# adajel/knp-emi-fenics-x

Hardware: AMD Instinct MI355X
Metric: assembled dofs/s (volume + membrane-facet assembly + membrane ODE sweep) per timestep; 3D idealized mesh, fp64 (higher is better)
Workload: dtype f64

## Files before the change

knp-emi-fenics-x_amd/csrc/kernels_assemble.hip:

```cpp
#include "knpemi_internal.h"

#define KN_ROW_STORE(v, p) __builtin_nontemporal_store((v), (p))

namespace {

__device__ __forceinline__ int logical_block(int bid, int nb) {
  const int q = nb >> 3, r = nb & 7, xcd = bid & 7, idx = bid >> 3;
  return xcd * q + (xcd < r ? xcd : r) + idx;
}

struct Rec {
  double x, y, z, c[KN_MAXK], phi;
};

__device__ __forceinline__ Rec load_rec(const double* __restrict__ VR, int v) {
  const double4* p = reinterpret_cast<const double4*>(VR) + 2 * (size_t)v;
  const double4 a = p[0], b = p[1];
  Rec r;
  r.x = a.x; r.y = a.y; r.z = a.z; r.c[0] = b.x; r.c[1] = b.y; r.c[2] = b.z; r.c[3] = a.w; r.phi = b.w;
  return r;
}

template <int NF>
__device__ __forceinline__ double facet_measure(const Rec (&p)[NF]) {
// ... 1361 lines not shown
    }
  }
#pragma unroll
  for (int m = 1; m < KN_MEM_LQ; m <<= 1)
#pragma unroll
    for (int a = 0; a < NF; ++a)
#pragma unroll
      for (int k = 0; k < KN_MAXK - 1; ++k) acc[a][k] += __shfl_xor(acc[a][k], m);
  if (live && lq == 0) {
#pragma unroll
    for (int a = 0; a < NF; ++a)
#pragma unroll
      for (int k = 0; k < KN_MAXK - 1; ++k)
        if (k < KS) D.gam_e[(size_t)KS * pos[a] + k] = acc[a][k];
  }
}

template <int NF>
__global__ __launch_bounds__(256) void knp_membrane_kernel(KnDev D, const KnConsts* __restrict__ Cp, int splitting) {
  extern __shared__ double qt[];
  knp_membrane_block<NF>(D, *Cp, splitting, logical_block(blockIdx.x, gridDim.x), nullptr, qt);
}

template <int NF>
__global__ __launch_bounds__(256) void emi_writeback_membrane_kernel(KnDev D, const KnConsts* __restrict__ Cp, int splitting,
                                                                     int nbm, const double* __restrict__ x, int n,
                                                                     const double* __restrict__ part, int np, double inv_n,
                                                                     double* __restrict__ mean_out) {
  extern __shared__ double qt[];
  if ((int)blockIdx.x < nbm) {
    knp_membrane_block<NF>(D, *Cp, splitting, logical_block(blockIdx.x, nbm), x, qt);
    return;
  }
  const int vb = blockIdx.x - nbm, nvb = gridDim.x - nbm;
  int i = vb * 256 + threadIdx.x;
  double xi = i < n ? x[i] : 0.0;
  double mean = 0.0;
  if (np > 0) {
    double v0 = 0.0, v1 = 0.0, v2 = 0.0, v3 = 0.0;
    const int t = threadIdx.x;
    if (t < np) v0 = part[t];
    if (t + 256 < np) v1 = part[t + 256];
    if (t + 512 < np) v2 = part[t + 512];
    if (t + 768 < np) v3 = part[t + 768];
    double sum = ((v0 + v1) + v2) + v3;
#pragma unroll
    for (int m = 32; m >= 1; m >>= 1) sum += __shfl_xor(sum, m);
    __shared__ double sh[4];
    if ((t & 63) == 0) sh[t >> 6] = sum;
    __syncthreads();
    mean = ((sh[0] + sh[1]) + (sh[2] + sh[3])) * inv_n;
    if (vb == 0 && t == 0 && mean_out) *mean_out = mean;
  }
  while (i < n) {
    D.VR[(size_t)i * KN_REC + 7] = xi - mean;
    i += nvb * 256;
    if (i < n) xi = x[i];
// ... 166 lines not shown
                            double* __restrict__ buf) {
  const int i = blockIdx.x * blockDim.x + threadIdx.x;
  if (i >= n) return;
  const int g = idx[i];
  if (kind == 0) {
    double* rec = D.VR + (size_t)g * KN_REC + 3;
    double* b = buf + (size_t)i * 5;
#pragma unroll
    for (int c = 0; c < 5; ++c) {
      if (pack) b[c] = rec[c];
      else rec[c] = b[c];
    }
  } else {
    const int w = 1 + KN_MAXK * n_slots;
    double* b = buf + (size_t)i * w;
    if (pack) b[0] = D.phiM[g];
    else D.phiM[g] = b[0];
    for (int c = 0; c < KN_MAXK * n_slots; ++c) {
      double* f = D.Ich + (size_t)c * D.NQtot + g;
      if (pack) b[1 + c] = *f;
      else *f = b[1 + c];
    }
  }
}

template <int NF, int LPR>
__global__ __launch_bounds__(256) void emi_membrane_rhs_kernel(KnDev D, const KnConsts* __restrict__ Cp, int splitting) {
  const KnConsts& C = *Cp;
  const int t = blockIdx.x * blockDim.x + threadIdx.x;
  const int mm = t / LPR, sub = t % LPR;
  const bool live = mm < D.M;
  const int m = live ? mm : D.M - 1;
  const int g = D.mrow[m];
  const bool cell_side = g >= C.voff[1];
  double gam = 0.0;
  for (int e = D.mptr[m] + sub; e < D.mptr[m + 1]; e += LPR) {
    const int ms = D.me_model[e];
    if (ms < 0) continue;
    gam += (cell_side ? 1.0 : -1.0) * C.C_phi * emi_membrane_entry_rhs<NF>(D, C, e, ms, splitting);
  }
#pragma unroll
  for (int k = 1; k < LPR; k <<= 1) gam += __shfl_xor(gam, k);
  if (live && sub == 0) D.b_emi[g] = D.b_emi[g] + gam;
}

int check_launch(const char* what) {
  hipError_t e = hipGetLastError();
  if (e != hipSuccess) {
    kn_set_error(std::string(what) + ": " + hipGetErrorString(e));
    return KNPEMI_EHIP;
  }
  return KNPEMI_OK;
}

template <class K>
int set_lds_limit(K kernel, size_t bytes) {
  if (bytes > 64 * 1024) {
    hipError_t e = hipFuncSetAttribute(reinterpret_cast<const void*>(kernel),
                                       hipFuncAttributeMaxDynamicSharedMemorySize, (int)bytes);
    if (e != hipSuccess) {
      kn_set_error(std::string("hipFuncSetAttribute(max dynamic LDS): ") + hipGetErrorString(e));
      return KNPEMI_EHIP;
    }
  }
  return KNPEMI_OK;
}
// ... 152 lines not shown
  const KnDev& D = h->dev;
  dim3 grid((n_entries + 255) / 256), block(256);
  const int v_cells = h->voff[1];
  if (h->NF == 2) hipLaunchKernelGGL(membrane_mass_kernel<2>, grid, block, 0, h->stream, D, n_entries, v_cells, d_entry_row, d_out);
  else if (h->NF == 3) hipLaunchKernelGGL(membrane_mass_kernel<3>, grid, block, 0, h->stream, D, n_entries, v_cells, d_entry_row, d_out);
  else hipLaunchKernelGGL(membrane_mass_kernel<4>, grid, block, 0, h->stream, D, n_entries, v_cells, d_entry_row, d_out);
  return check_launch("membrane_mass_kernel");
}

int kn_launch_knp_membrane(knpemi_handle* h, int flags) {
  const KnDev& D = h->dev;
  if (D.nftot == 0) return KNPEMI_OK;
  const int split = (flags & KNPEMI_NO_SPLITTING) ? 0 : 1;
  const int NF = h->NF;
  const size_t lds = (size_t)D.nq_gamma * (1 + NF + (NF == 4 ? 2 * NF : 0)) * sizeof(double);
  dim3 grid((2 * (size_t)D.nftot * KN_MEM_LQ + 255) / 256), block(256);
  KnProfScope prof(h, KNPEMI_K_KNP_MEMBRANE);
  if (NF == 2) hipLaunchKernelGGL((knp_membrane_kernel<2>), grid, block, lds, h->cur, D, h->d_consts, split);
  else if (NF == 3) hipLaunchKernelGGL((knp_membrane_kernel<3>), grid, block, lds, h->cur, D, h->d_consts, split);
  else hipLaunchKernelGGL((knp_membrane_kernel<4>), grid, block, lds, h->cur, D, h->d_consts, split);
  return check_launch("knp_membrane_kernel");
}

int kn_launch_emi_writeback_membrane(knpemi_handle* h, const double* x, const double* part, int np, double inv_n, double* mean_out) {
  const KnDev& D = h->dev;
  const int n = D.Ntot;
  if (n == 0) return KNPEMI_OK;
  const int split = (h->emi_flags & KNPEMI_NO_SPLITTING) ? 0 : 1;
  const int NF = h->NF;
  const size_t lds = (size_t)D.nq_gamma * (1 + NF + (NF == 4 ? 2 * NF : 0)) * sizeof(double);
  const int nbm = (int)((2 * (size_t)D.nftot * KN_MEM_LQ + 255) / 256);
  const int nbv = std::max(1, std::min(1024, (n + 255) / 256));
  dim3 grid(nbm + nbv), block(256);
  KnProfScope prof(h, KNPEMI_K_KNP_MEMBRANE);
  if (NF == 2) hipLaunchKernelGGL((emi_writeback_membrane_kernel<2>), grid, block, lds, h->cur, D, h->d_consts, split, nbm, x, n, part, np, inv_n, mean_out);
  else if (NF == 3) hipLaunchKernelGGL((emi_writeback_membrane_kernel<3>), grid, block, lds, h->cur, D, h->d_consts, split, nbm, x, n, part, np, inv_n, mean_out);
  else hipLaunchKernelGGL((emi_writeback_membrane_kernel<4>), grid, block, lds, h->cur, D, h->d_consts, split, nbm, x, n, part, np, inv_n, mean_out);
  return check_launch("emi_writeback_membrane_kernel");
}

int kn_launch_knp_membrane_pre(knpemi_handle* h, int flags) {
  const KnDev& D = h->dev;
  if (D.nftot == 0) return KNPEMI_OK;
  const int split = (flags & KNPEMI_NO_SPLITTING) ? 0 : 1;
  const int NF = h->NF;
  const size_t lds = (size_t)D.nq_gamma * (1 + NF + (NF == 4 ? 2 * NF : 0)) * sizeof(double);
  dim3 grid((2 * D.nftot + 255) / 256), block(256);
  KnProfScope prof(h, KNPEMI_K_KNP_MEMBRANE);
  if (NF == 2) hipLaunchKernelGGL((knp_membrane_pre_kernel<2>), grid, block, lds, h->cur, D, h->d_consts, split);
  else if (NF == 3) hipLaunchKernelGGL((knp_membrane_pre_kernel<3>), grid, block, lds, h->cur, D, h->d_consts, split);
  else hipLaunchKernelGGL((knp_membrane_pre_kernel<4>), grid, block, lds, h->cur, D, h->d_consts, split);
  return check_launch("knp_membrane_pre_kernel");
}

int kn_launch_emi_membrane_rhs(knpemi_handle* h, int flags) {
  const KnDev& D = h->dev;
  if (D.M == 0) return KNPEMI_OK;
  const int split = (flags & KNPEMI_NO_SPLITTING) ? 0 : 1;
  const int lpr = h->lpr;
  dim3 grid(((size_t)D.M * lpr + 255) / 256), block(256);
// ... 62 lines not shown
```

knp-emi-fenics-x_amd/csrc/knpemi_api.hip:

```cpp
#include <algorithm>
#include <array>
#include <cstdlib>
#include <cstring>
#include <numeric>

#include "knpemi_internal.h"

static thread_local std::string g_err;
void kn_set_error(const std::string& msg) { g_err = msg; }

extern "C" const char* knpemi_last_error(void) { return g_err.c_str(); }

extern "C" int knpemi_device_count(void) {
  int n = 0;
  if (hipGetDeviceCount(&n) != hipSuccess) return 0;
  return n;
}

namespace {

template <class T>
int dev_upload(knpemi_handle* h, const std::vector<T>& v, const T** out) {
  void* p = nullptr;
  size_t bytes = std::max<size_t>(v.size(), 1) * sizeof(T);
// ... 1072 lines not shown
  const int nq = h->n_q[sub], ne = h->n_vert[0], ni = h->n_vert[sub];
  if (nq == 0) return KNPEMI_OK;
  if ((size_t)ne + ni + 2 * (size_t)nq > h->stage_len) return fail(KNPEMI_EINVAL, "knpemi_trace: staging buffer too small");
  KN_HIP(hipSetDevice(h->device));
  double* de = h->d_stage;
  double* di = de + ne;
  double* qe = di + ni;
  double* qi = qe + nq;
  KN_HIP(hipMemcpyAsync(de, u_e, (size_t)ne * sizeof(double), hipMemcpyHostToDevice, h->stream));
  KN_HIP(hipMemcpyAsync(di, u_i, (size_t)ni * sizeof(double), hipMemcpyHostToDevice, h->stream));
  int rc = kn_launch_trace(h, de, di, sub, qe, qi);
  if (rc) return rc;
  KN_HIP(hipMemcpyAsync(q_e, qe, (size_t)nq * sizeof(double), hipMemcpyDeviceToHost, h->stream));
  KN_HIP(hipMemcpyAsync(q_i, qi, (size_t)nq * sizeof(double), hipMemcpyDeviceToHost, h->stream));
  KN_HIP(hipStreamSynchronize(h->stream));
  return KNPEMI_OK;
}

extern "C" int knpemi_assemble_emi(knpemi_handle* h, int flags) {
  if (!h) return fail(KNPEMI_EINVAL, "null handle");
  if (!h->have_params) return fail(KNPEMI_EINVAL, "knpemi_assemble_emi: knpemi_set_params not called");
  KN_HIP(hipSetDevice(h->device));
  h->emi_flags = flags;
  if (flags & KNPEMI_ON_AUX_STREAM) {
    KN_HIP(hipEventRecord(h->ev_fork, h->stream));
    KN_HIP(hipStreamWaitEvent(h->aux, h->ev_fork, 0));
    h->cur = h->aux;
    int rc = kn_launch_emi_rows(h, flags);
    h->cur = h->stream;
    if (rc) return rc;
    KN_HIP(hipEventRecord(h->ev_join, h->aux));
    return KNPEMI_OK;
  }
  return kn_launch_emi_rows(h, flags);
}

extern "C" int knpemi_join(knpemi_handle* h) {
  if (!h) return fail(KNPEMI_EINVAL, "null handle");
  KN_HIP(hipSetDevice(h->device));
  KN_HIP(hipStreamWaitEvent(h->stream, h->ev_join, 0));
  KN_HIP(hipStreamWaitEvent(h->stream, h->ev_join2, 0));
  return KNPEMI_OK;
}

extern "C" int knpemi_assemble_emi_membrane_rhs(knpemi_handle* h, int flags) {
  if (!h) return fail(KNPEMI_EINVAL, "null handle");
  if (!h->have_params) return fail(KNPEMI_EINVAL, "knpemi_assemble_emi_membrane_rhs: knpemi_set_params not called");
  KN_HIP(hipSetDevice(h->device));
  return kn_launch_emi_membrane_rhs(h, flags);
}

extern "C" int knpemi_assemble_knp_membrane_early(knpemi_handle* h, int flags) {
  if (!h) return fail(KNPEMI_EINVAL, "null handle");
  if (!h->have_params) return fail(KNPEMI_EINVAL, "knpemi_assemble_knp_membrane_early: knpemi_set_params not called");
  KN_HIP(hipSetDevice(h->device));
  int rc;
  if (flags & KNPEMI_ON_AUX_STREAM) {
    KN_HIP(hipEventRecord(h->ev_pre_fork, h->stream));
    KN_HIP(hipStreamWaitEvent(h->aux, h->ev_pre_fork, 0));
    h->cur = h->aux;
    rc = kn_launch_knp_membrane_pre(h, flags);
    h->cur = h->stream;
    if (rc) return rc;
    KN_HIP(hipEventRecord(h->ev_pre, h->aux));
    h->pre_pending = 1;
    return KNPEMI_OK;
  }
  return kn_launch_knp_membrane_pre(h, flags);
}

extern "C" int knpemi_assemble_knp(knpemi_handle* h, int flags) {
  if (!h) return fail(KNPEMI_EINVAL, "null handle");
  if (!h->have_params) return fail(KNPEMI_EINVAL, "knpemi_assemble_knp: knpemi_set_params not called");
  KN_HIP(hipSetDevice(h->device));
  KN_HIP(hipStreamWaitEvent(h->stream, h->ev_join, 0));
  KN_HIP(hipStreamWaitEvent(h->stream, h->ev_join2, 0));
  if (flags & KNPEMI_MEMBRANE_EARLY) {
    if (h->pre_pending) {
      KN_HIP(hipStreamWaitEvent(h->stream, h->ev_pre, 0));
      h->pre_pending = 0;
    }
    return kn_launch_knp_rows(h, flags);
  }
  if (!h->fuse_membrane) {
    const int split = (flags & KNPEMI_NO_SPLITTING) ? 0 : 1;
    if (!kn_gam_current(h, split)) {
      int rc = kn_launch_knp_membrane(h, flags);
      if (rc) return rc;
    }
  }
  return kn_launch_knp_rows(h, flags);
}

extern "C" int knpemi_solve_emi(knpemi_handle* h, double rtol, double atol, int maxit, int* iters, double* relres) {
  if (!h) return fail(KNPEMI_EINVAL, "null handle");
  if (!(rtol >= 0) || !(atol >= 0) || maxit < 0) return fail(KNPEMI_EINVAL, "knpemi_solve_emi: bad tolerances");
  kn_inputs_changed(h);
  KN_HIP(hipSetDevice(h->device));
  KN_HIP(hipStreamWaitEvent(h->stream, h->ev_join, 0));
  KN_HIP(hipStreamWaitEvent(h->stream, h->ev_join2, 0));
  return kn_solve_emi(h, rtol, atol, maxit, iters, relres);
}

extern "C" int knpemi_solve_knp(knpemi_handle* h, double rtol, double atol, int maxit, int* iters, double* relres) {
  if (!h) return fail(KNPEMI_EINVAL, "null handle");
  if (!(rtol >= 0) || !(atol >= 0) || maxit < 0) return fail(KNPEMI_EINVAL, "knpemi_solve_knp: bad tolerances");
  kn_inputs_changed(h);
  KN_HIP(hipSetDevice(h->device));
  KN_HIP(hipStreamWaitEvent(h->stream, h->ev_join, 0));
  KN_HIP(hipStreamWaitEvent(h->stream, h->ev_join2, 0));
  return kn_solve_knp(h, rtol, atol, maxit, iters, relres);
}

extern "C" int knpemi_extrapolate_guess(knpemi_handle* h, int which) {
  if (!h) return fail(KNPEMI_EINVAL, "null handle");
  if (which != KNPEMI_B_EMI && which != KNPEMI_B_KNP) return fail(KNPEMI_EINVAL, "knpemi_extrapolate_guess: unknown system");
  kn_inputs_changed(h);
  KN_HIP(hipSetDevice(h->device));
  return kn_extrapolate_guess(h, which);
}

extern "C" int knpemi_solver_setup(knpemi_handle* h, int which, int precond, double theta) {
  if (!h) return fail(KNPEMI_EINVAL, "null handle");
  if (which != KNPEMI_B_EMI && which != KNPEMI_B_KNP) return fail(KNPEMI_EINVAL, "knpemi_solver_setup: unknown system");
  if (precond != KNPEMI_PC_JACOBI && precond != KNPEMI_PC_AMG)
    return fail(KNPEMI_EINVAL, "knpemi_solver_setup: unknown preconditioner");
  KnAmg& G = which == KNPEMI_B_EMI ? h->amg_emi : h->amg_knp;
  (which == KNPEMI_B_EMI ? h->pc_emi : h->pc_knp) = precond;
  G.cfg.theta = theta > 0 ? theta : 0.08;
  G.built = false;
  return KNPEMI_OK;
}

// ... 59 lines not shown
}

extern "C" int knpemi_get_csr_values(knpemi_handle* h, int which, double* vals) {
  if (!h || !vals) return fail(KNPEMI_EINVAL, "knpemi_get_csr_values: null argument");
  const double* src; size_t n;
  if (which == KNPEMI_A_EMI) { src = h->dev.A_emi; n = h->dev.nnz; }
  else if (which == KNPEMI_P_EMI) { src = h->dev.P_emi; n = h->dev.nnz; }
  else if (which == KNPEMI_A_KNP) { src = h->dev.A_knp; n = (size_t)(h->K - 1) * h->dev.nnzL; }
  else return fail(KNPEMI_EINVAL, "knpemi_get_csr_values: unknown matrix");
  KN_HIP(hipSetDevice(h->device));
  KN_HIP(hipMemcpyAsync(vals, src, n * sizeof(double), hipMemcpyDeviceToHost, h->stream));
  KN_HIP(hipStreamSynchronize(h->stream));
  return KNPEMI_OK;
}

extern "C" int knpemi_set_csr_values(knpemi_handle* h, int which, const double* vals) {
  if (!h || !vals) return fail(KNPEMI_EINVAL, "knpemi_set_csr_values: null argument");
  double* dst; size_t n;
  if (which == KNPEMI_A_EMI) { dst = h->dev.A_emi; n = h->dev.nnz; }
  else if (which == KNPEMI_P_EMI) { dst = h->dev.P_emi; n = h->dev.nnz; }
  else if (which == KNPEMI_A_KNP) { dst = h->dev.A_knp; n = (size_t)(h->K - 1) * h->dev.nnzL; }
  else return fail(KNPEMI_EINVAL, "knpemi_set_csr_values: unknown matrix");
  KN_HIP(hipSetDevice(h->device));
  KN_HIP(hipStreamWaitEvent(h->stream, h->ev_join, 0));
  KN_HIP(hipMemcpyAsync(dst, vals, n * sizeof(double), hipMemcpyHostToDevice, h->stream));
  KN_HIP(hipStreamSynchronize(h->stream));
  return KNPEMI_OK;
}

extern "C" int knpemi_set_rhs(knpemi_handle* h, int which, const double* b) {
  if (!h || !b) return fail(KNPEMI_EINVAL, "knpemi_set_rhs: null argument");
  double* dst; size_t n;
  if (which == KNPEMI_B_EMI) { dst = h->dev.b_emi; n = h->dev.Ntot; }
  else if (which == KNPEMI_B_KNP) { dst = h->dev.b_knp; n = (size_t)(h->K - 1) * h->dev.Ntot; }
  else return fail(KNPEMI_EINVAL, "knpemi_set_rhs: unknown vector");
  KN_HIP(hipSetDevice(h->device));
  KN_HIP(hipStreamWaitEvent(h->stream, h->ev_join, 0));
  KN_HIP(hipMemcpyAsync(dst, b, n * sizeof(double), hipMemcpyHostToDevice, h->stream));
  KN_HIP(hipStreamSynchronize(h->stream));
  return KNPEMI_OK;
}

extern "C" int knpemi_device_rhs(knpemi_handle* h, int which, const double** b) {
  if (!h || !b) return fail(KNPEMI_EINVAL, "null argument");
  if (which == KNPEMI_B_EMI) *b = h->dev.b_emi;
  else if (which == KNPEMI_B_KNP) *b = h->dev.b_knp;
  else return fail(KNPEMI_EINVAL, "knpemi_device_rhs: unknown vector");
  return KNPEMI_OK;
}

extern "C" int knpemi_get_rhs(knpemi_handle* h, int which, double* b) {
  if (!h || !b) return fail(KNPEMI_EINVAL, "knpemi_get_rhs: null argument");
  const double* src; size_t n;
  if (which == KNPEMI_B_EMI) { src = h->dev.b_emi; n = h->dev.Ntot; }
  else if (which == KNPEMI_B_KNP) { src = h->dev.b_knp; n = (size_t)(h->K - 1) * h->dev.Ntot; }
  else return fail(KNPEMI_EINVAL, "knpemi_get_rhs: unknown vector");
  KN_HIP(hipSetDevice(h->device));
  KN_HIP(hipMemcpyAsync(b, src, n * sizeof(double), hipMemcpyDeviceToHost, h->stream));
  KN_HIP(hipStreamSynchronize(h->stream));
  return KNPEMI_OK;
}

extern "C" int knpemi_set_solution(knpemi_handle* h, int which, const double* x, int on_device) {
  if (!h || !x) return fail(KNPEMI_EINVAL, "knpemi_set_solution: null argument");
  kn_inputs_changed(h);
  KN_HIP(hipSetDevice(h->device));
  const hipMemcpyKind kind = on_device ? hipMemcpyDeviceToDevice : hipMemcpyHostToDevice;
  KnDev& D = h->dev;
  if (which == KNPEMI_B_EMI) {
    const double* src = x;
    if (!on_device) {
      KN_HIP(hipMemcpyAsync(h->d_stage, x, (size_t)D.Ntot * sizeof(double), kind, h->stream));
      src = h->d_stage;
    }
    if (on_device && h->fold_membrane && h->have_params && !h->fuse_membrane && !h->dist.on) {
      KN_HIP(hipStreamWaitEvent(h->stream, h->ev_join, 0));
      KN_HIP(hipStreamWaitEvent(h->stream, h->ev_join2, 0));
      if (int rc = kn_launch_emi_writeback_membrane(h, src, nullptr, 0, 0.0, nullptr)) return rc;
      kn_gam_formed(h, (h->emi_flags & KNPEMI_NO_SPLITTING) ? 0 : 1);
    } else if (int rc = kn_launch_field_scatter(h, src, D.VR + 7, D.Ntot, KN_REC)) return rc;
  } else if (which == KNPEMI_B_KNP) {
    const int KS = h->K - 1;
    if (on_device) {
      if (!h->have_params) return fail(KNPEMI_EINVAL, "knpemi_set_solution: knpemi_set_params not called");
      int rc = h->fuse_update ? kn_launch_knp_writeback_update(h, x) : kn_launch_knp_order(h, const_cast<double*>(x), 0);
      if (rc) return rc;
    } else
    for (int s = 0; s < h->n_sub; ++s)
      for (int k = 0; k < KS; ++k) {
        const size_t nv = h->n_vert[s];
        if (!nv) continue;
        KN_HIP(hipMemcpyAsync(D.csol + (size_t)k * D.Ntot + h->voff[s],
                              x + (size_t)KS * h->voff[s] + (size_t)k * nv, nv * sizeof(double), kind, h->stream));
      }
  } else return fail(KNPEMI_EINVAL, "knpemi_set_solution: unknown system");
  if (!on_device && which == KNPEMI_B_KNP && h->fuse_update) {
    if (!h->have_params) return fail(KNPEMI_EINVAL, "knpemi_set_solution: knpemi_set_params not called");
    int rc = kn_launch_update_pde(h);
    if (rc) return rc;
  }
  if (!on_device) KN_HIP(hipStreamSynchronize(h->stream));
  return KNPEMI_OK;
}

extern "C" int knpemi_get_solution(knpemi_handle* h, int which, double* x) {
// ... 160 lines not shown
  KnOdeModel& m = h->ode[slot];
  for (int i = 0; i < 3 * h->K; ++i)
    if (ion_param[i] < 0 || ion_param[i] >= m.n_params)
      return fail(KNPEMI_EINVAL, "knpemi_ode_step: parameter index out of range");
  if (v_index < 0 || v_index >= m.n_states) return fail(KNPEMI_EINVAL, "knpemi_ode_step: bad V index");
  const bool fixed = m.method != KNPEMI_ODE_LSODA;
  if (!(dt > 0) || (!fixed && (!(rtol >= 0) || !(atol >= 0) || (rtol == 0 && atol == 0))))
    return fail(KNPEMI_EINVAL, "knpemi_ode_step: bad dt / tolerances");
  if (h->ode_only && (flags & (KNPEMI_ODE_SET_TRACES | KNPEMI_ODE_SET_V)))
    return fail(KNPEMI_EINVAL, "knpemi_ode_step: a handle of knpemi_ode_create has no PDE fields to read");
  kn_inputs_changed(h);
  KN_HIP(hipSetDevice(h->device));
  if (flags & (KNPEMI_ODE_ON_AUX_STREAM | KNPEMI_ODE_ON_AUX2_STREAM)) {
    const bool second = (flags & KNPEMI_ODE_ON_AUX2_STREAM) != 0;
    hipStream_t side = second ? h->aux2 : h->aux;
    KN_HIP(hipEventRecord(h->ev_fork, h->stream));
    KN_HIP(hipStreamWaitEvent(side, h->ev_fork, 0));
    h->cur = side;
    int rc = fixed ? kn_launch_ode_fixed_step(h, slot, t0, dt, flags, ion_param, v_index)
                   : kn_launch_ode_step(h, slot, t0, dt, rtol, atol, flags, ion_param, v_index);
    h->cur = h->stream;
    if (rc) return rc;
    KN_HIP(hipEventRecord(second ? h->ev_join2 : h->ev_join, side));
    return KNPEMI_OK;
  }
  if (fixed) return kn_launch_ode_fixed_step(h, slot, t0, dt, flags, ion_param, v_index);
  return kn_launch_ode_step(h, slot, t0, dt, rtol, atol, flags, ion_param, v_index);
}

extern "C" int knpemi_ode_advance(knpemi_handle* h, int sub, int model, double t0, double dt, int n_steps, double rtol,
                                  double atol, const int32_t* rec_idx, int n_rec, int every, double* history,
                                  const knpemi_ode_ss* ss, int32_t* steps_taken, int32_t* failed_step) {
  int slot = ode_slot(h, sub, model, 1);
  if (slot < 0) return KNPEMI_EINVAL;
  const KnOdeModel& m = h->ode[slot];
  const bool fixed = m.method != KNPEMI_ODE_LSODA;
  if (n_steps < 0 || !(dt > 0) || (!fixed && (!(rtol >= 0) || !(atol >= 0) || (rtol == 0 && atol == 0))))
    return fail(KNPEMI_EINVAL, "knpemi_ode_advance: bad n_steps / dt / tolerances");
  if (history) {
    if (every < 1 || n_rec < 1 || n_rec > 8 || !rec_idx)
      return fail(KNPEMI_EINVAL, "knpemi_ode_advance: recording needs every >= 1 and 1..8 state indices");
    for (int i = 0; i < n_rec; ++i)
      if (rec_idx[i] < 0 || rec_idx[i] >= m.n_states)
        return fail(KNPEMI_EINVAL, "knpemi_ode_advance: recorded state index out of range");
  } else {
    every = 1;
// ... 58 lines not shown
    return fail(KNPEMI_EODE, "the fixed-step integrator left a non-finite state on at least one membrane dof");
  if (st[2]) return fail(KNPEMI_EODE, "LSODA failed on at least one membrane dof (odeSolver.py:121 `assert success`)");
  return KNPEMI_OK;
}

extern "C" int knpemi_debug_ode_stamps(knpemi_handle* h, int sub, int model, uint64_t* out, int max_blocks) {
  int slot = ode_slot(h, sub, model, 1);
  if (slot < 0) return KNPEMI_EINVAL;
  KnOdeModel& m = h->ode[slot];
  if (!m.d_stamps || !out) return fail(KNPEMI_EINVAL, "knpemi_debug_ode_stamps: run with KNPEMI_ODE_STAMPS=1");
  const int nb = std::min(max_blocks, m.n_stat_blocks - 1);
  KN_HIP(hipSetDevice(h->device));
  KN_HIP(hipStreamSynchronize(h->aux));
  KN_HIP(hipStreamSynchronize(h->stream));
  KN_HIP(hipMemcpy(out, m.d_stamps, (size_t)nb * 24 * sizeof(uint64_t), hipMemcpyDeviceToHost));
  return nb;
}

extern "C" int knpemi_update_pde(knpemi_handle* h) {
  if (!h) return fail(KNPEMI_EINVAL, "null handle");
  if (!h->have_params) return fail(KNPEMI_EINVAL, "knpemi_update_pde: knpemi_set_params not called");
  kn_inputs_changed(h);
  KN_HIP(hipSetDevice(h->device));
  return kn_launch_update_pde(h);
}

int kn_observe_chunk();

namespace {
void observe_free(knpemi_handle* h) {
  for (void* p : h->obs.allocs) (void)hipFree(p);
  h->obs = knpemi_handle::KnObserve{};
}

template <class T>
int obs_upload(knpemi_handle* h, const T* src, size_t n, T** out) {
  void* p = nullptr;
  KN_HIP(hipMalloc(&p, std::max<size_t>(n, 1) * sizeof(T)));
  h->obs.allocs.push_back(p);
  if (n) KN_HIP(hipMemcpy(p, src, n * sizeof(T), hipMemcpyHostToDevice));
  *out = static_cast<T*>(p);
  return 0;
}
}

namespace {
// ... 365 lines not shown
```

knp-emi-fenics-x_amd/csrc/knpemi_internal.h:

```cpp
#pragma once

#include <hip/hip_runtime.h>
#include "block_spmv.h"
#include <stdint.h>

#include <cstring>
#include <functional>
#include <memory>
#include <string>
#include <unordered_map>
#include <vector>

#include "../../include/knpemi_hip.h"

#define KN_MAXK KNPEMI_MAX_IONS
#define KN_MAXSUB KNPEMI_MAX_SUB
#define KN_REC 8
#define KN_CSLOT(k) ((k) < 3 ? 4 + (k) : 3)
#define KN_BLOCK 256
#define KN_SLICE 64
#define KN_CHUNK_SIMPLEX 16
#define KN_CHUNK_HEX 8

struct KnSubConst {
// ... 184 lines not shown
};
#define KN_COARSE_MAX 64
#define KN_COARSE_OFF 8

struct KnVecPlan {
  bool set = false;
  const int32_t* send_idx = nullptr; const int32_t* recv_idx = nullptr;
  int n_send = 0, n_recv = 0;
  double* send_buf = nullptr; double* recv_buf = nullptr;
  std::vector<int32_t> peer;
  std::vector<int64_t> send_off, send_cnt, recv_off, recv_cnt;
};

struct knpemi_handle {
  int device = 0;
  hipStream_t stream = nullptr;
  hipStream_t aux = nullptr;
  hipStream_t aux2 = nullptr;
  hipEvent_t ev_join2 = nullptr;
  hipEvent_t ev_pre_fork = nullptr, ev_pre = nullptr;
  int pre_pending = 0;
  hipStream_t cur = nullptr;
  hipEvent_t ev_fork = nullptr, ev_join = nullptr;
  hipEvent_t ev0 = nullptr, ev1 = nullptr;
  int gdim = 0, cell_kind = 0, NV = 0, NF = 0, n_sub = 0, K = 0;
  std::vector<int> n_vert, n_cell, n_q, n_facet, n_models;
  std::vector<int> voff, coff, qoff, foff, moff;
  KnConsts consts{};
  KnConsts* d_consts = nullptr;
  const void* d_lsoda_coef = nullptr;
  KnDev dev{};
  int have_params = 0;
  int lpr = 1;
  bool hex_affine = false;
  bool tet_uniform = false;
  bool hex_uniform = false;
  KnHexGeo hex_geo{};
  int lds_doubles_emi = 0, lds_doubles_knp = 0;
  int lds_uniq_max = 0;
  std::vector<void*> allocs;
  std::vector<void*> rtc_modules;
  std::vector<KnOdeModel> ode;
  bool ode_only = false;
  std::vector<int> h_rowptr, h_colind, h_rowptrL, h_colindL;
  void* comm = nullptr;
  int comm_rank = 0, comm_world = 1;
// ... 9 lines not shown
  double* fused_part = nullptr; size_t fused_part_n = 0;
  double* guess_old[2] = {nullptr, nullptr};
  int guess_have[2] = {0, 0};
  KnAmg amg_emi, amg_knp;
  struct KnGraph { hipGraphExec_t exec = nullptr; uint64_t key = 0; };
  KnGraph graph_emi, graph_knp;
  std::unordered_map<uint64_t, hipGraphExec_t> fused_graphs;
  struct FusedMode { bool decided = false, graph = true; int solves = 0; double t[2] = {0.0, 0.0}; int n[2] = {0, 0}; };
  FusedMode fused_mode[2];
  int pc_emi = KNPEMI_PC_AMG, pc_knp = KNPEMI_PC_AMG;
  int fuse_update = 0;
  int knp_min_it = 0;
  int emi_norm_pre = 0;
  int knp_method = 0;
  double* gm_V = nullptr; size_t gm_n = 0;
  double* gm_state = nullptr;
  bool plain_knp = false;
  int fuse_membrane = 0;
  uint64_t inputs_gen = 1;
  uint64_t gam_gen = 0;
  int gam_split = 1;
  int fold_membrane = 1;
  int emi_flags = 0;
  int prof_stride = 1;
  unsigned prof_count[16] = {0};
  int lds_gam_max = 0;
  bool blocks_clustered = false;
  KnDist dist;
  struct KnObserve {
    int n_obs = 0, n_blk = 0, capacity = 0;
    int4* blk = nullptr;
    int* blk_ptr = nullptr;
    int* op = nullptr;
    int* stride = nullptr;
    const double** base = nullptr;
    double* denom = nullptr;
    int* idx = nullptr;
    double* w = nullptr;
    double* part = nullptr;
    unsigned long long* ctl = nullptr;
    double* rows = nullptr;
    double* xbuf = nullptr;
    int rank = 0, world = 1;
    knpemi_allreduce_fn allreduce = nullptr;
    void* ctx = nullptr;
    std::vector<void*> allocs;
// ... 17 lines not shown
      hipEvent_t a, b;
      if (hipEventCreate(&a) != hipSuccess || hipEventCreate(&b) != hipSuccess) { on = false; return; }
      v.push_back(a); v.push_back(b);
    }
    (void)hipEventRecord(v[h->prof_used[k]], h->cur);
  }
  ~KnProfScope() {
    if (!on) return;
    (void)hipEventRecord(h->prof_ev[k][h->prof_used[k] + 1], h->cur);
    h->prof_used[k] += 2;
  }
};

void kn_set_error(const std::string& msg);
#define KN_HIP(call)                                                                     \
  do {                                                                                   \
    hipError_t e_ = (call);                                                              \
    if (e_ != hipSuccess) {                                                              \
      kn_set_error(std::string(#call) + ": " + hipGetErrorString(e_));                   \
      return KNPEMI_EHIP;                                                                \
    }                                                                                    \
  } while (0)

struct OdeDev;
struct OdeArgs;
int kn_launch_ode_raw(hipStream_t st, int model_id, const OdeDev& dv, const OdeArgs& a, const void* coef);
int kn_lsoda_coef_upload(void** out);
void kn_comm_destroy(knpemi_handle* h);
int kn_comm_create(int device, int rank, int world, const char* id_bytes, size_t len, void** out);
void kn_comm_free(void* comm);
int kn_comm_sendrecv(void* comm, int world, int device, hipStream_t stream, const double* send_buf_dev, double* recv_buf_dev,
                     int n_parts, const int32_t* peer, const int64_t* send_off, const int64_t* send_cnt,
                     const int64_t* recv_off, const int64_t* recv_cnt);
int kn_gamma_quadrature(int NF, std::vector<double>* out);

int kn_launch_emi_rows(knpemi_handle* h, int flags);
int kn_launch_knp_rows(knpemi_handle* h, int flags);
int kn_launch_knp_membrane_pre(knpemi_handle* h, int flags);
int kn_launch_emi_membrane_rhs(knpemi_handle* h, int flags);
int kn_launch_knp_membrane(knpemi_handle* h, int flags);
int kn_launch_emi_writeback_membrane(knpemi_handle* h, const double* x, const double* part, int np, double inv_n, double* mean_out);
int kn_launch_membrane_mass(knpemi_handle* h, int n_entries, const int* d_entry_row, double* d_out);
int kn_launch_ode_step(knpemi_handle* h, int slot, double t0, double dt, double rtol, double atol,
                       int flags, const int32_t* ion_param, int v_index);
int kn_launch_update_pde(knpemi_handle* h);
int kn_launch_observe(knpemi_handle* h);
int kn_launch_observe_combine(knpemi_handle* h);
int kn_rtc_bind(knpemi_handle* h, KnOdeModel& m, int n_states, int n_params, const char* rhs_source);
int kn_rtc_launch(knpemi_handle* h, const KnOdeModel& m, const void* dev_view, size_t dev_bytes, const void* args,
                  size_t args_bytes, const void* coef);
int kn_rtc_advance_launch(knpemi_handle* h, const KnOdeModel& m, const void* args, size_t args_bytes, const void* adv,
                          size_t adv_bytes, const void* coef);
int kn_launch_ode_fixed_step(knpemi_handle* h, int slot, double t0, double dt, int flags, const int32_t* ion_param,
                             int v_index);
int kn_launch_ode_fixed_advance(knpemi_handle* h, const KnOdeModel& m, const void* args, const void* adv);
int kn_rtc_fixed_launch(knpemi_handle* h, const KnOdeModel& m, const void* dev_view, const void* args);
int kn_rtc_fixed_advance_launch(knpemi_handle* h, const KnOdeModel& m, const void* args, const void* adv);
int kn_ode_advance(knpemi_handle* h, int slot, double t0, double dt, int n_steps, double rtol, double atol,
                   const int32_t* rec_idx, int n_rec, int every, double* history, const knpemi_ode_ss* ss,
                   int32_t* steps_taken, int32_t* failed_step);
int kn_solve_emi(knpemi_handle* h, double rtol, double atol, int maxit, int* iters, double* relres);
int kn_solve_knp(knpemi_handle* h, double rtol, double atol, int maxit, int* iters, double* relres);
int kn_extrapolate_guess(knpemi_handle* h, int which);
int kn_launch_knp_order(knpemi_handle* h, double* x, int to_blocks);
// ... 7 lines not shown
```

knp-emi-fenics-x_amd/knpemi/stepper.py:

```python
from __future__ import annotations

import ctypes as C

import numpy as np

from . import _lib as L


class DeviceStepper:
    def __init__(self, forms_emi, forms_knp, c, c_prev, phi, phi_M_prev, solve_emi=None, solve_knp=None,
                 assemble_knp_twice=False, overlap=True, device_solves=None, extrapolate_guess=True,
                 fuse_update=None, fuse_membrane=False, early_membrane=False, knp_method="gmres",
                 ode_method="lsoda", ode_substeps=None):
        a = forms_emi[0]
        self.dp = a.dp
        self.a = a
        self.lib = self.dp.lib
        self.c, self.c_prev, self.phi, self.phi_M_prev = c, c_prev, phi, phi_M_prev
        if device_solves is not None:
            rtol_emi, rtol_knp = device_solves
            self.iterations = []
            from .pdeSolver import set_emi_solver_options, set_knp_solver_options
            set_knp_solver_options(a.dp, knp_method)
            set_emi_solver_options(a.dp, "preconditioned" if knp_method == "gmres" else "true")
# ... 155 lines not shown
        if calibrate:
            L.check(lib.knpemi_profile(dp.h, (1 << L.KERNEL_NAMES.index("ode_step_kernel"))
                                       | (1 << L.KERNEL_NAMES.index("emi_rows_kernel"))))
        ode_aux = bool(self.overlap and self.ode_on_aux)
        if self.overlap and not ode_aux:
            L.check(lib.knpemi_assemble_emi(dp.h, self.flags_emi | L.SKIP_MEMBRANE_RHS | L.ON_AUX_STREAM))
        side_of_sub = {}
        for m in self.models:
            if m._sub not in side_of_sub:
                side_of_sub[m._sub] = L.ODE_ON_AUX2 if side_of_sub else (L.ODE_ON_AUX if ode_aux else 0)
        for wanted in (L.ODE_ON_AUX2, L.ODE_ON_AUX, 0):
            for m in self.models:
                if side_of_sub[m._sub] != wanted:
                    continue
                L.check(lib.knpemi_ode_step(dp.h, m._sub, m._model, float(m.time), self.dt, m.rtol, m.atol,
                                            flags | wanted, L.iptr(m._ion_param), int(m.V_index)))
                m.time = m.time + self.dt
        if ode_aux:
            L.check(lib.knpemi_assemble_emi(dp.h, self.flags_emi | L.SKIP_MEMBRANE_RHS))
        if len(side_of_sub) > 1 and not self.overlap:
            L.check(lib.knpemi_join(dp.h))
        if self.overlap:
            L.check(lib.knpemi_join(dp.h))
            L.check(lib.knpemi_assemble_emi_membrane_rhs(dp.h, self.flags_emi))
            if calibrate:
                us = {}
                for name in ("ode_step_kernel", "emi_rows_kernel"):
                    n, ms = C.c_int64(), C.c_double()
                    L.check(lib.knpemi_profile_read(dp.h, L.KERNEL_NAMES.index(name), C.byref(n), C.byref(ms)))
                    us[name] = ms.value
                L.check(lib.knpemi_profile(dp.h, 0))
                self.ode_on_aux = us["emi_rows_kernel"] > us["ode_step_kernel"]
                if min(us.values()) < self.overlap_threshold_ms:
                    self.overlap = False
        else:
            L.check(lib.knpemi_assemble_emi(dp.h, self.flags_emi))
        knp_flags = self.flags_knp
        if self.early_membrane:
            L.check(lib.knpemi_assemble_knp_membrane_early(dp.h, self.flags_knp | (L.ON_AUX_STREAM if self.overlap else 0)))
            knp_flags |= L.MEMBRANE_EARLY
        if self.solve_emi is not None:
            self.solve_emi(dp)
            if halo is not None:
                halo.exchange_bulk()
        L.check(lib.knpemi_assemble_knp(dp.h, knp_flags))
        if self.assemble_knp_twice:
            L.check(lib.knpemi_assemble_knp(dp.h, knp_flags))
# ... 26 lines not shown
```

Measured before the change: 797.6 million.

## Defer EMI membrane Robin RHS and fold it into writeback-membrane launch

The membrane Robin contribution to b_emi is no longer launched right after the join. It is marked pending and later settled, either fused as extra blocks into the emi_writeback_membrane kernel or launched lazily before anything consumes b_emi. Stream waits on the side-stream join events are also skipped when no side work is pending. This removes a separate kernel launch and some redundant event waits per timestep, at the cost of more involved state tracking that could miss a consumer of b_emi.

```diff
diff --git a/knp-emi-fenics-x_amd/csrc/kernels_assemble.hip b/knp-emi-fenics-x_amd/csrc/kernels_assemble.hip
--- a/knp-emi-fenics-x_amd/csrc/kernels_assemble.hip
+++ b/knp-emi-fenics-x_amd/csrc/kernels_assemble.hip
@@ -1407,9 +1407,34 @@
   knp_membrane_block<NF>(D, *Cp, splitting, logical_block(blockIdx.x, gridDim.x), nullptr, qt);
 }
 
-template <int NF>
+template <int NF, int LPR>
+__device__ __forceinline__ void emi_membrane_rhs_block(const KnDev& D, const KnConsts& C, int splitting, int blk) {
+  const int t = blk * 256 + threadIdx.x;
+  const int mm = t / LPR, sub = t % LPR;
+  const bool live = mm < D.M;
+  const int m = live ? mm : D.M - 1;
+  const int g = D.mrow[m];
+  const bool cell_side = g >= C.voff[1];
+  double gam = 0.0;
+  for (int e = D.mptr[m] + sub; e < D.mptr[m + 1]; e += LPR) {
+    const int ms = D.me_model[e];
+    if (ms < 0) continue;
+    gam += (cell_side ? 1.0 : -1.0) * C.C_phi * emi_membrane_entry_rhs<NF>(D, C, e, ms, splitting);
+  }
+#pragma unroll
+  for (int k = 1; k < LPR; k <<= 1) gam += __shfl_xor(gam, k);
+  if (live && sub == 0) D.b_emi[g] = D.b_emi[g] + gam;
+}
+
+template <int NF, int LPR>
+__global__ __launch_bounds__(256) void emi_membrane_rhs_kernel(KnDev D, const KnConsts* __restrict__ Cp, int splitting) {
+  emi_membrane_rhs_block<NF, LPR>(D, *Cp, splitting, blockIdx.x);
+}
+
+template <int NF, int LPR>
 __global__ __launch_bounds__(256) void emi_writeback_membrane_kernel(KnDev D, const KnConsts* __restrict__ Cp, int splitting,
-                                                                     int nbm, const double* __restrict__ x, int n,
+                                                                     int nbm, int nvb, int robin_splitting,
+                                                                     const double* __restrict__ x, int n,
                                                                      const double* __restrict__ part, int np, double inv_n,
                                                                      double* __restrict__ mean_out) {
   extern __shared__ double qt[];
@@ -1417,7 +1442,11 @@
     knp_membrane_block<NF>(D, *Cp, splitting, logical_block(blockIdx.x, nbm), x, qt);
     return;
   }
-  const int vb = blockIdx.x - nbm, nvb = gridDim.x - nbm;
+  const int vb = blockIdx.x - nbm;
+  if (LPR > 0 && vb >= nvb) {
+    emi_membrane_rhs_block<NF, (LPR > 0 ? LPR : 1)>(D, *Cp, robin_splitting, vb - nvb);
+    return;
+  }
   int i = vb * 256 + threadIdx.x;
   double xi = i < n ? x[i] : 0.0;
   double mean = 0.0;
@@ -1630,26 +1659,6 @@
       else *f = b[1 + c];
     }
   }
-}
-
-template <int NF, int LPR>
-__global__ __launch_bounds__(256) void emi_membrane_rhs_kernel(KnDev D, const KnConsts* __restrict__ Cp, int splitting) {
-  const KnConsts& C = *Cp;
-  const int t = blockIdx.x * blockDim.x + threadIdx.x;
-  const int mm = t / LPR, sub = t % LPR;
-  const bool live = mm < D.M;
-  const int m = live ? mm : D.M - 1;
-  const int g = D.mrow[m];
-  const bool cell_side = g >= C.voff[1];
-  double gam = 0.0;
-  for (int e = D.mptr[m] + sub; e < D.mptr[m + 1]; e += LPR) {
-    const int ms = D.me_model[e];
-    if (ms < 0) continue;
-    gam += (cell_side ? 1.0 : -1.0) * C.C_phi * emi_membrane_entry_rhs<NF>(D, C, e, ms, splitting);
-  }
-#pragma unroll
-  for (int k = 1; k < LPR; k <<= 1) gam += __shfl_xor(gam, k);
-  if (live && sub == 0) D.b_emi[g] = D.b_emi[g] + gam;
 }
 
 int check_launch(const char* what) {
@@ -1848,7 +1857,8 @@
   return check_launch("knp_membrane_kernel");
 }
 
-int kn_launch_emi_writeback_membrane(knpemi_handle* h, const double* x, const double* part, int np, double inv_n, double* mean_out) {
+int kn_launch_emi_writeback_membrane(knpemi_handle* h, const double* x, const double* part, int np, double inv_n, double* mean_out,
+                                     int robin_split) {
   const KnDev& D = h->dev;
   const int n = D.Ntot;
   if (n == 0) return KNPEMI_OK;
@@ -1857,11 +1867,19 @@
   const size_t lds = (size_t)D.nq_gamma * (1 + NF + (NF == 4 ? 2 * NF : 0)) * sizeof(double);
   const int nbm = (int)((2 * (size_t)D.nftot * KN_MEM_LQ + 255) / 256);
   const int nbv = std::max(1, std::min(1024, (n + 255) / 256));
-  dim3 grid(nbm + nbv), block(256);
+  const bool robin = robin_split >= 0 && D.M > 0;
+  const int lpr = robin ? h->lpr : 0;
+  const int nbr = robin ? (int)(((size_t)D.M * lpr + 255) / 256) : 0;
+  dim3 grid(nbm + nbv + nbr), block(256);
   KnProfScope prof(h, KNPEMI_K_KNP_MEMBRANE);
-  if (NF == 2) hipLaunchKernelGGL((emi_writeback_membrane_kernel<2>), grid, block, lds, h->cur, D, h->d_consts, split, nbm, x, n, part, np, inv_n, mean_out);
-  else if (NF == 3) hipLaunchKernelGGL((emi_writeback_membrane_kernel<3>), grid, block, lds, h->cur, D, h->d_consts, split, nbm, x, n, part, np, inv_n, mean_out);
-  else hipLaunchKernelGGL((emi_writeback_membrane_kernel<4>), grid, block, lds, h->cur, D, h->d_consts, split, nbm, x, n, part, np, inv_n, mean_out);
+#define KN_WB(NFV, L) hipLaunchKernelGGL((emi_writeback_membrane_kernel<NFV, L>), grid, block, lds, h->cur, D, h->d_consts, split, \
+                                         nbm, nbv, robin_split, x, n, part, np, inv_n, mean_out)
+#define KN_WB_L(NFV) \
+  switch (lpr) { case 0: KN_WB(NFV, 0); break; case 1: KN_WB(NFV, 1); break; case 2: KN_WB(NFV, 2); break; \
+                 case 8: KN_WB(NFV, 8); break; default: KN_WB(NFV, 4); }
+  if (NF == 2) { KN_WB_L(2) } else if (NF == 3) { KN_WB_L(3) } else { KN_WB_L(4) }
+#undef KN_WB_L
+#undef KN_WB
   return check_launch("emi_writeback_membrane_kernel");
 }
 
diff --git a/knp-emi-fenics-x_amd/csrc/knpemi_api.hip b/knp-emi-fenics-x_amd/csrc/knpemi_api.hip
--- a/knp-emi-fenics-x_amd/csrc/knpemi_api.hip
+++ b/knp-emi-fenics-x_amd/csrc/knpemi_api.hip
@@ -1118,6 +1118,8 @@
   if (!h->have_params) return fail(KNPEMI_EINVAL, "knpemi_assemble_emi: knpemi_set_params not called");
   KN_HIP(hipSetDevice(h->device));
   h->emi_flags = flags;
+  h->robin_pending = (flags & KNPEMI_SKIP_MEMBRANE_RHS) ? 1 : 0;
+  h->robin_split = (flags & KNPEMI_NO_SPLITTING) ? 0 : 1;
   if (flags & KNPEMI_ON_AUX_STREAM) {
     KN_HIP(hipEventRecord(h->ev_fork, h->stream));
     KN_HIP(hipStreamWaitEvent(h->aux, h->ev_fork, 0));
@@ -1126,6 +1128,7 @@
     h->cur = h->stream;
     if (rc) return rc;
     KN_HIP(hipEventRecord(h->ev_join, h->aux));
+    h->side_pending |= 1;
     return KNPEMI_OK;
   }
   return kn_launch_emi_rows(h, flags);
@@ -1134,16 +1137,24 @@
 extern "C" int knpemi_join(knpemi_handle* h) {
   if (!h) return fail(KNPEMI_EINVAL, "null handle");
   KN_HIP(hipSetDevice(h->device));
-  KN_HIP(hipStreamWaitEvent(h->stream, h->ev_join, 0));
-  KN_HIP(hipStreamWaitEvent(h->stream, h->ev_join2, 0));
-  return KNPEMI_OK;
-}
+  if (int rc = kn_wait_side(h)) return rc;
+  return KNPEMI_OK;
+}
+
+static int kn_settle_robin(knpemi_handle* h, int split) {
+  if (!h->robin_pending) return KNPEMI_OK;
+  if (!h->have_params) return fail(KNPEMI_EINVAL, "membrane Robin term of b_emi pending: knpemi_set_params not called");
+  if (int rc = kn_wait_side(h)) return rc;
+  h->robin_pending = 0;
+  return kn_launch_emi_membrane_rhs(h, split ? 0 : KNPEMI_NO_SPLITTING);
+}
+static int kn_settle_robin(knpemi_handle* h) { return kn_settle_robin(h, h->robin_split); }
 
 extern "C" int knpemi_assemble_emi_membrane_rhs(knpemi_handle* h, int flags) {
   if (!h) return fail(KNPEMI_EINVAL, "null handle");
   if (!h->have_params) return fail(KNPEMI_EINVAL, "knpemi_assemble_emi_membrane_rhs: knpemi_set_params not called");
   KN_HIP(hipSetDevice(h->device));
-  return kn_launch_emi_membrane_rhs(h, flags);
+  return kn_settle_robin(h, (flags & KNPEMI_NO_SPLITTING) ? 0 : 1);
 }
 
 extern "C" int knpemi_assemble_knp_membrane_early(knpemi_handle* h, int flags) {
@@ -1169,8 +1180,7 @@
   if (!h) return fail(KNPEMI_EINVAL, "null handle");
   if (!h->have_params) return fail(KNPEMI_EINVAL, "knpemi_assemble_knp: knpemi_set_params not called");
   KN_HIP(hipSetDevice(h->device));
-  KN_HIP(hipStreamWaitEvent(h->stream, h->ev_join, 0));
-  KN_HIP(hipStreamWaitEvent(h->stream, h->ev_join2, 0));
+  if (int rc = kn_wait_side(h)) return rc;
   if (flags & KNPEMI_MEMBRANE_EARLY) {
     if (h->pre_pending) {
       KN_HIP(hipStreamWaitEvent(h->stream, h->ev_pre, 0));
@@ -1193,8 +1203,8 @@
   if (!(rtol >= 0) || !(atol >= 0) || maxit < 0) return fail(KNPEMI_EINVAL, "knpemi_solve_emi: bad tolerances");
   kn_inputs_changed(h);
   KN_HIP(hipSetDevice(h->device));
-  KN_HIP(hipStreamWaitEvent(h->stream, h->ev_join, 0));
-  KN_HIP(hipStreamWaitEvent(h->stream, h->ev_join2, 0));
+  if (int rc = kn_wait_side(h)) return rc;
+  if (int rc = kn_settle_robin(h)) return rc;
   return kn_solve_emi(h, rtol, atol, maxit, iters, relres);
 }
 
@@ -1203,8 +1213,8 @@
   if (!(rtol >= 0) || !(atol >= 0) || maxit < 0) return fail(KNPEMI_EINVAL, "knpemi_solve_knp: bad tolerances");
   kn_inputs_changed(h);
   KN_HIP(hipSetDevice(h->device));
-  KN_HIP(hipStreamWaitEvent(h->stream, h->ev_join, 0));
-  KN_HIP(hipStreamWaitEvent(h->stream, h->ev_join2, 0));
+  if (int rc = kn_wait_side(h)) return rc;
+  if (int rc = kn_settle_robin(h)) return rc;
   return kn_solve_knp(h, rtol, atol, maxit, iters, relres);
 }
 
@@ -1310,7 +1320,7 @@
   else if (which == KNPEMI_A_KNP) { dst = h->dev.A_knp; n = (size_t)(h->K - 1) * h->dev.nnzL; }
   else return fail(KNPEMI_EINVAL, "knpemi_set_csr_values: unknown matrix");
   KN_HIP(hipSetDevice(h->device));
-  KN_HIP(hipStreamWaitEvent(h->stream, h->ev_join, 0));
+  if (int rc = kn_wait_side(h, false)) return rc;
   KN_HIP(hipMemcpyAsync(dst, vals, n * sizeof(double), hipMemcpyHostToDevice, h->stream));
   KN_HIP(hipStreamSynchronize(h->stream));
   return KNPEMI_OK;
@@ -1323,7 +1333,8 @@
   else if (which == KNPEMI_B_KNP) { dst = h->dev.b_knp; n = (size_t)(h->K - 1) * h->dev.Ntot; }
   else return fail(KNPEMI_EINVAL, "knpemi_set_rhs: unknown vector");
   KN_HIP(hipSetDevice(h->device));
-  KN_HIP(hipStreamWaitEvent(h->stream, h->ev_join, 0));
+  if (which == KNPEMI_B_EMI) h->robin_pending = 0;
+  if (int rc = kn_wait_side(h, false)) return rc;
   KN_HIP(hipMemcpyAsync(dst, b, n * sizeof(double), hipMemcpyHostToDevice, h->stream));
   KN_HIP(hipStreamSynchronize(h->stream));
   return KNPEMI_OK;
@@ -1331,7 +1342,11 @@
 
 extern "C" int knpemi_device_rhs(knpemi_handle* h, int which, const double** b) {
   if (!h || !b) return fail(KNPEMI_EINVAL, "null argument");
-  if (which == KNPEMI_B_EMI) *b = h->dev.b_emi;
+  if (which == KNPEMI_B_EMI) {
+    KN_HIP(hipSetDevice(h->device));
+    if (int rc = kn_settle_robin(h)) return rc;
+    *b = h->dev.b_emi;
+  }
   else if (which == KNPEMI_B_KNP) *b = h->dev.b_knp;
   else return fail(KNPEMI_EINVAL, "knpemi_device_rhs: unknown vector");
   return KNPEMI_OK;
@@ -1344,6 +1359,10 @@
   else if (which == KNPEMI_B_KNP) { src = h->dev.b_knp; n = (size_t)(h->K - 1) * h->dev.Ntot; }
   else return fail(KNPEMI_EINVAL, "knpemi_get_rhs: unknown vector");
   KN_HIP(hipSetDevice(h->device));
+  if (which == KNPEMI_B_EMI) {
+    if (int rc = kn_settle_robin(h)) return rc;
+    if (int rc = kn_wait_side(h, false)) return rc;
+  }
   KN_HIP(hipMemcpyAsync(b, src, n * sizeof(double), hipMemcpyDeviceToHost, h->stream));
   KN_HIP(hipStreamSynchronize(h->stream));
   return KNPEMI_OK;
@@ -1362,13 +1381,19 @@
       src = h->d_stage;
     }
     if (on_device && h->fold_membrane && h->have_params && !h->fuse_membrane && !h->dist.on) {
-      KN_HIP(hipStreamWaitEvent(h->stream, h->ev_join, 0));
-      KN_HIP(hipStreamWaitEvent(h->stream, h->ev_join2, 0));
-      if (int rc = kn_launch_emi_writeback_membrane(h, src, nullptr, 0, 0.0, nullptr)) return rc;
+      if (int rc = kn_wait_side(h)) return rc;
+      const int robin = h->robin_pending ? h->robin_split : -1;
+      h->robin_pending = 0;
+      if (int rc = kn_launch_emi_writeback_membrane(h, src, nullptr, 0, 0.0, nullptr, robin)) return rc;
       kn_gam_formed(h, (h->emi_flags & KNPEMI_NO_SPLITTING) ? 0 : 1);
-    } else if (int rc = kn_launch_field_scatter(h, src, D.VR + 7, D.Ntot, KN_REC)) return rc;
+    } else {
+      if (int rc = kn_settle_robin(h)) return rc;
+      if (int rc = kn_launch_field_scatter(h, src, D.VR + 7, D.Ntot, KN_REC)) return rc;
+    }
   } else if (which == KNPEMI_B_KNP) {
     const int KS = h->K - 1;
+    if (h->fuse_update)
+      if (int rc = kn_settle_robin(h)) return rc;
     if (on_device) {
       if (!h->have_params) return fail(KNPEMI_EINVAL, "knpemi_set_solution: knpemi_set_params not called");
       int rc = h->fuse_update ? kn_launch_knp_writeback_update(h, x) : kn_launch_knp_order(h, const_cast<double*>(x), 0);
@@ -1575,6 +1600,7 @@
     h->cur = h->stream;
     if (rc) return rc;
     KN_HIP(hipEventRecord(second ? h->ev_join2 : h->ev_join, side));
+    h->side_pending |= second ? 2 : 1;
     return KNPEMI_OK;
   }
   if (fixed) return kn_launch_ode_fixed_step(h, slot, t0, dt, flags, ion_param, v_index);
@@ -1679,6 +1705,7 @@
   if (!h->have_params) return fail(KNPEMI_EINVAL, "knpemi_update_pde: knpemi_set_params not called");
   kn_inputs_changed(h);
   KN_HIP(hipSetDevice(h->device));
+  if (int rc = kn_settle_robin(h)) return rc;
   return kn_launch_update_pde(h);
 }
 
diff --git a/knp-emi-fenics-x_amd/csrc/knpemi_internal.h b/knp-emi-fenics-x_amd/csrc/knpemi_internal.h
--- a/knp-emi-fenics-x_amd/csrc/knpemi_internal.h
+++ b/knp-emi-fenics-x_amd/csrc/knpemi_internal.h
@@ -230,6 +230,7 @@
   int pre_pending = 0;
   hipStream_t cur = nullptr;
   hipEvent_t ev_fork = nullptr, ev_join = nullptr;
+  int side_pending = 0;
   hipEvent_t ev0 = nullptr, ev1 = nullptr;
   int gdim = 0, cell_kind = 0, NV = 0, NF = 0, n_sub = 0, K = 0;
   std::vector<int> n_vert, n_cell, n_q, n_facet, n_models;
@@ -285,6 +286,7 @@
   int gam_split = 1;
   int fold_membrane = 1;
   int emi_flags = 0;
+  int robin_pending = 0, robin_split = 1;
   int prof_stride = 1;
   unsigned prof_count[16] = {0};
   int lds_gam_max = 0;
@@ -348,6 +350,18 @@
     }                                                                                    \
   } while (0)
 
+inline int kn_wait_side(knpemi_handle* h, bool second = true) {
+  if (h->side_pending & 1) {
+    KN_HIP(hipStreamWaitEvent(h->stream, h->ev_join, 0));
+    h->side_pending &= ~1;
+  }
+  if (second && (h->side_pending & 2)) {
+    KN_HIP(hipStreamWaitEvent(h->stream, h->ev_join2, 0));
+    h->side_pending &= ~2;
+  }
+  return KNPEMI_OK;
+}
+
 struct OdeDev;
 struct OdeArgs;
 int kn_launch_ode_raw(hipStream_t st, int model_id, const OdeDev& dv, const OdeArgs& a, const void* coef);
@@ -365,7 +379,8 @@
 int kn_launch_knp_membrane_pre(knpemi_handle* h, int flags);
 int kn_launch_emi_membrane_rhs(knpemi_handle* h, int flags);
 int kn_launch_knp_membrane(knpemi_handle* h, int flags);
-int kn_launch_emi_writeback_membrane(knpemi_handle* h, const double* x, const double* part, int np, double inv_n, double* mean_out);
+int kn_launch_emi_writeback_membrane(knpemi_handle* h, const double* x, const double* part, int np, double inv_n, double* mean_out,
+                                     int robin_split = -1);
 int kn_launch_membrane_mass(knpemi_handle* h, int n_entries, const int* d_entry_row, double* d_out);
 int kn_launch_ode_step(knpemi_handle* h, int slot, double t0, double dt, double rtol, double atol,
                        int flags, const int32_t* ion_param, int v_index);
diff --git a/knp-emi-fenics-x_amd/knpemi/stepper.py b/knp-emi-fenics-x_amd/knpemi/stepper.py
--- a/knp-emi-fenics-x_amd/knpemi/stepper.py
+++ b/knp-emi-fenics-x_amd/knpemi/stepper.py
@@ -201,7 +201,6 @@
             L.check(lib.knpemi_join(dp.h))
         if self.overlap:
             L.check(lib.knpemi_join(dp.h))
-            L.check(lib.knpemi_assemble_emi_membrane_rhs(dp.h, self.flags_emi))
             if calibrate:
                 us = {}
                 for name in ("ode_step_kernel", "emi_rows_kernel"):
```

Result: no change. 799.3 million (median of 5 runs) (+0.2%).
